# WHU-USI3DV/LaneMapping

Measured on AMD Instinct MI355X. Metric: BEV tiles/sec end-to-end (LAS points -> polylines), higher is better.
Workload: dtype f32; 1 GPU; on-GPU LAS->BEV raster (4,194,304 points/tile resident in HBM) + configs/Proj_polyline_fpn_vit_vertex_2.py, batch=16 per GPU, seeded random weights; lines_per_tile=45, streams=2, hip_graphs=True, points=resident, stream_check=not run (--full runs it), gather_check=n/a (1 rank), raster_check=not run (--full runs it), dist_ranks=1, rccl_ranks=1

## Files before the change

### include/lanemap_hip.h

```cpp
#ifndef LANEMAP_HIP_H
#define LANEMAP_HIP_H
#include <stdint.h>
#ifdef __cplusplus
extern "C" {
#endif

enum { LM_OK = 0, LM_ERR_ARG = 1, LM_ERR_HIP = 2, LM_ERR_NO_DEVICE = 3, LM_ERR_CAPACITY = 4 };
enum { LM_ACT_NONE = 0, LM_ACT_RELU = 1, LM_ACT_GELU = 2 };

int lm_abi_version(void);
const char* lm_last_error(void);
int lm_device_count(void);

int lm_conv2d_nhwc_mfma_f32(void* stream, const float* x, int ldx, const float* wp, int CoutP,
                            const float* scale, const float* shift, const float* res, int ldr, int res_rows,
                            float* y, int ldy, int B, int H, int W, int Cin, int Cout, int KH, int KW,
                            int stride, int pad_h, int pad_w, int dil, int act);
int lm_conv2d_nhwc_mfma_resup_f32(void* stream, const float* x, int ldx, const float* wp, int CoutP, const float* scale,
                                  const float* shift, const float* res_coarse, int ldr, int Hr, int Wr, float* y, int ldy,
                                  int B, int H, int W, int Cin, int Cout, int KH, int KW, int stride, int pad_h, int pad_w,
                                  int dil, int act);

int lm_winograd44_supported(int H, int W, int Cin, int dil);
int lm_winograd44_gn_chunks(int H, int W, int dil);
// ... 4 lines not shown
                              int Cin, int Cout, int dil, int act, double* gn_partial);
int lm_conv3x3_winograd44_twin_f32(void* stream, const float* x, int ldx, const float* wu, int CoutP, const float* scale,
                                   const float* shift, const float* res, int ldr, float* y, int ldy, int B, int H, int W,
                                   int Cin, int Cout, int dil, int act, void* workspace, long workspace_bytes);
int lm_wino44_split_fragments(void* stream, const float* frag, float* out, long n_quads);
int lm_conv3x3_winograd44_split_f32(void* stream, const float* x, int ldx, const float* wu_split, int CoutP, const float* scale,
                                    const float* shift, const float* res, int ldr, float* y, int ldy, int B, int H, int W,
                                    int Cin, int Cout, int dil, int act, double* gn_partial, float post);
int lm_conv3x3_winograd44_split_twin_f32(void* stream, const float* x, int ldx, const float* wu, int CoutP, const float* scale,
                                         const float* shift, const float* res, int ldr, float* y, int ldy, int B, int H, int W,
                                         int Cin, int Cout, int dil, int act, void* workspace, long workspace_bytes, float post);

int lm_conv2d_nhwc_mfma_f32_gnstats(void* stream, const float* x, int ldx, const float* wp, int CoutP, const float* shift,
                                    float* y, int ldy, double* gn_partial, int B, int H, int W, int Cin, int Cout,
                                    int KH, int KW, int stride, int pad_h, int pad_w, int dil);
int lm_gn_finalize(void* stream, const double* partial, float* stats, int B, int HW, int C, int nchunk, float eps);
int lm_gn_finalize_split(void* stream, const double* partial, float* stats, int B, int HW, int C, int nchunk, float eps, int split);

int lm_stem_conv7x7_bn_relu(void* stream, const float* x_chw, const float* w_k64, const float* scale,
                            const float* shift, float* y_nhwc, int B, int H, int W);
int lm_stem_conv7x7_bn_relu_u8(void* stream, const unsigned char* x_hwc3, const float* w_k64, const float* scale,
                               const float* shift, float* y_nhwc, int B, int H, int W);
int lm_maxpool3x3s2_nhwc(void* stream, const float* x, float* y, int B, int H, int W, int C);
int lm_conv2d_nhwc_small(void* stream, const float* x, int ldx, const float* w_tc16, const float* scale,
                         const float* shift, float* y, int ldy, int B, int H, int W, int Cin, int Cout,
                         int KH, int KW, int stride, int pad_h, int pad_w, int pre_relu, int act);

int lm_gn_stats(void* stream, const float* x, double* workspace, float* stats, int B, int HW, int C, float eps);
long lm_gn_stats_workspace_bytes(int B, int HW, int C);
int lm_gn_relu_upsample(void* stream, const float* x, const float* stats, const float* gamma, const float* beta,
                        float* y, int B, int Hi, int Wi, int Ho, int Wo, int C, int accumulate);
int lm_gn_relu_upsample_sum(void* stream, int n, const float* const* x, const float* const* stats, const int* Hi, const int* Wi,
                            const int* ldx , const float* gamma, const float* beta,
                            float* y, int B, int Ho, int Wo, int C);
int lm_gn_relu_upsample_sum_conv1x1(void* stream, int n, const float* const* x, const float* const* stats, const int* Hi, const int* Wi,
                                    const int* ldx, const float* gamma, const float* beta, float* y, int B, int Ho, int Wo, int C,
                                    const float* w_c16, const float* bias, int cout, float* y1, int ldy1);
int lm_upsample_bilinear_nhwc(void* stream, const float* x, int ldx, const float* add, int lda, float* y, int ldy,
                              int B, int Hi, int Wi, int Ho, int Wo, int C);
int lm_upsample_bilinear_to_chw(void* stream, const float* x, int ldx, float* y_chw, int B, int Hi, int Wi,
                                int Ho, int Wo, int C);
int lm_layernorm_rows(void* stream, const float* x, const float* gamma, const float* beta, float* y,
                      long rows, int D, float eps);
int lm_unpatchify(void* stream, const float* tokens, float* y_nhwc, int B, int G, int P, int C);
int lm_token_mix_mfma_f32(void* stream, const float* x, const float* wt, int ldw, const float* bias, const float* res, float* y,
                          int B, int M, int K, int N, int act);
// ... 142 lines not shown
```

### lanemapping_amd/_lib.py

```python
import ctypes as C
import os

_HERE = os.path.dirname(os.path.abspath(__file__))
LIB_PATH = os.environ.get('LANEMAP_HIP_LIB') or os.path.join(_HERE, 'liblanemap_hip.so')

c_f32p = C.POINTER(C.c_float)
vp, i32, i64, f32 = C.c_void_p, C.c_int, C.c_long, C.c_float


class LmRasterParams(C.Structure):
    _fields_ = [('quat', C.c_float * 4), ('trans', C.c_float * 3), ('bev_img_offset', C.c_float * 2),
                ('img_reso', C.c_float * 2), ('local_min_ele', C.c_float), ('ele_reso', C.c_float),
                ('inten_lo', C.c_float), ('inten_hi', C.c_float)]


class LmLasHeader(C.Structure):
    _fields_ = [('version_major', C.c_int), ('version_minor', C.c_int), ('point_format', C.c_int), ('record_len', C.c_int),
                ('n_points', C.c_long), ('offset_to_points', C.c_long), ('scale', C.c_double * 3), ('offset', C.c_double * 3),
                ('min_xyz', C.c_double * 3), ('max_xyz', C.c_double * 3)]


class LmStripGrid(C.Structure):
    _fields_ = [('x0', C.c_double), ('y0', C.c_double), ('cell', C.c_double), ('nx', C.c_int), ('ny', C.c_int)]

# ... 5 lines not shown
SIGNATURES = {
    'lm_abi_version': (i32, []),
    'lm_last_error': (C.c_char_p, []),
    'lm_device_count': (i32, []),
    'lm_conv2d_nhwc_mfma_f32': (i32, [vp, vp, i32, vp, i32, vp, vp, vp, i32, i32, vp, i32,
                                      i32, i32, i32, i32, i32, i32, i32, i32, i32, i32, i32, i32]),
    'lm_conv2d_nhwc_mfma_resup_f32': (i32, [vp, vp, i32, vp, i32, vp, vp, vp, i32, i32, i32, vp, i32,
                                            i32, i32, i32, i32, i32, i32, i32, i32, i32, i32, i32, i32]),
    'lm_winograd44_supported': (i32, [i32, i32, i32, i32]),
    'lm_winograd44_gn_chunks': (i32, [i32, i32, i32]),
    'lm_winograd44_tiles': (i64, [i32, i32, i32, i32]),
    'lm_winograd44_twin_workspace_bytes': (i64, [i32, i32, i32, i32, i32, i32]),
    'lm_conv3x3_winograd44_f32': (i32, [vp, vp, i32, vp, i32, vp, vp, vp, i32, vp, i32, i32, i32, i32, i32, i32, i32, i32, vp]),
    'lm_conv3x3_winograd44_twin_f32': (i32, [vp, vp, i32, vp, i32, vp, vp, vp, i32, vp, i32, i32, i32, i32, i32, i32, i32, i32, vp, i64]),
    'lm_wino44_split_fragments': (i32, [vp, vp, vp, i64]),
    'lm_conv3x3_winograd44_split_f32': (i32, [vp, vp, i32, vp, i32, vp, vp, vp, i32, vp, i32, i32, i32, i32, i32, i32, i32, i32, vp, f32]),
    'lm_conv3x3_winograd44_split_twin_f32': (i32, [vp, vp, i32, vp, i32, vp, vp, vp, i32, vp, i32, i32, i32, i32, i32, i32, i32, i32, vp, i64, f32]),
    'lm_conv2d_nhwc_mfma_f32_gnstats': (i32, [vp, vp, i32, vp, i32, vp, vp, i32, vp] + [i32] * 11),
    'lm_gn_finalize': (i32, [vp, vp, vp, i32, i32, i32, i32, f32]),
    'lm_gn_finalize_split': (i32, [vp, vp, vp, i32, i32, i32, i32, f32, i32]),
    'lm_stem_conv7x7_bn_relu': (i32, [vp, vp, vp, vp, vp, vp, i32, i32, i32]),
    'lm_stem_conv7x7_bn_relu_u8': (i32, [vp, vp, vp, vp, vp, vp, i32, i32, i32]),
    'lm_maxpool3x3s2_nhwc': (i32, [vp, vp, vp, i32, i32, i32, i32]),
    'lm_conv2d_nhwc_small': (i32, [vp, vp, i32, vp, vp, vp, vp, i32, i32, i32, i32, i32, i32, i32, i32, i32, i32, i32, i32, i32]),
    'lm_gn_stats': (i32, [vp, vp, vp, vp, i32, i32, i32, f32]),
    'lm_gn_stats_workspace_bytes': (i64, [i32, i32, i32]),
    'lm_gn_relu_upsample': (i32, [vp, vp, vp, vp, vp, vp, i32, i32, i32, i32, i32, i32, i32]),
    'lm_gn_relu_upsample_sum': (i32, [vp, i32, vp, vp, vp, vp, vp, vp, vp, vp, i32, i32, i32, i32]),
    'lm_gn_relu_upsample_sum_conv1x1': (i32, [vp, i32, vp, vp, vp, vp, vp, vp, vp, vp, i32, i32, i32, i32, vp, vp, i32, vp, i32]),
    'lm_upsample_bilinear_nhwc': (i32, [vp, vp, i32, vp, i32, vp, i32, i32, i32, i32, i32, i32, i32]),
    'lm_upsample_bilinear_to_chw': (i32, [vp, vp, i32, vp, i32, i32, i32, i32, i32, i32]),
    'lm_layernorm_rows': (i32, [vp, vp, vp, vp, vp, i64, i32, f32]),
    'lm_token_mix_mfma_f32': (i32, [vp, vp, vp, i32, vp, vp, vp, i32, i32, i32, i32, i32]),
    'lm_unpatchify': (i32, [vp, vp, vp, i32, i32, i32, i32]),
    'lm_attention_f32': (i32, [vp, vp, vp, i32, i32, i32, i32, f32]),
    'lm_attention_masked_f32': (i32, [vp, vp, vp, vp, i32, i32, i32, i32, f32]),
    'lm_head_tokens': (i32, [vp, vp, vp, vp, f32, i32, i32, i32, i32, i32, i32]),
    'lm_head_tokens_window': (i32, [vp, vp, vp, i32, i32, i32, i32, i32, i32]),
    'lm_head_stage2': (i32, [vp, vp, i32, i32, vp, vp, vp, vp, vp, i64]),
    'lm_head_proposal_conf': (i32, [vp, vp, vp, vp, vp, i32, i32]),
    'lm_head_endpoint_tile': (i32, []),
    'lm_head_endpoint': (i32, [vp, vp, i32, vp, vp, vp, vp, vp, vp, vp, vp, i32, i32, i32, i32, i32]),
    'lm_decode_proposals': (i32, [vp, vp, vp, vp, vp, vp, vp, vp, vp, vp, i32, i32, i32, f32, i32, i32]),
    'lm_decode_orient': (i32, [vp, vp, i32, i32, vp, i64]),
    'lm_decode_semantic': (i32, [vp, vp, vp, vp, vp, i32, i32, i32, f32, i32]),
    'lm_endp_topk_workspace_bytes': (i64, [i32]),
# ... 85 lines not shown
```

### lanemapping_amd/csrc/conv_direct.hip

```cpp
#include "common.h"

#include <type_traits>

typedef float f32x4 __attribute__((ext_vector_type(4)));

namespace {

constexpr int ST = 16;
constexpr int SP = 2 * ST + 5;
constexpr int SPP = 40;

template <bool U8>
__global__ __launch_bounds__(256) void stem_kernel(const void* __restrict__ xin, const float* __restrict__ w,
                                                   const float* __restrict__ scale, const float* __restrict__ shift,
                                                   float* __restrict__ y, int H, int W, int Ho, int Wo) {
    __shared__ float in[3][SP][SPP];
    const int tid = threadIdx.x;
    const int b = blockIdx.z;
    const int oy0 = blockIdx.y * ST, ox0 = blockIdx.x * ST;
    const int iy0 = oy0 * 2 - 3, ix0 = ox0 * 2 - 3;
    for (int i = tid; i < 3 * SP * SP; i += 256) {
        const int c = i / (SP * SP), r = (i / SP) % SP, q = i % SP;
        const int iy = iy0 + r, ix = ix0 + q;
        float v = 0.f;
// ... 14 lines not shown
            for (int c = 0; c < 3; ++c) {
                const float v = in[c][2 * py + ky][2 * px + kx];
                const float* wr = w + ((ky * 7 + kx) * 3 + c) * 64;
#pragma unroll
                for (int q = 0; q < 64; ++q) acc[q] = fmaf(v, wr[q], acc[q]);
            }
    const int oy = oy0 + py, ox = ox0 + px;
    if (oy < Ho && ox < Wo) {
        f32x4* out = reinterpret_cast<f32x4*>(y + (((long)b * Ho + oy) * Wo + ox) * 64);
#pragma unroll
        for (int q = 0; q < 16; ++q) {
            f32x4 o;
#pragma unroll
            for (int e = 0; e < 4; ++e) o[e] = fmaxf(acc[4 * q + e] * scale[4 * q + e] + shift[4 * q + e], 0.f);
            out[q] = o;
        }
    }
}

constexpr int SMW = 112;
constexpr int SMJ = 77;
typedef float f32x16s __attribute__((ext_vector_type(16)));

template <bool U8>
__global__ __launch_bounds__(256, 2) void stem_mfma_kernel(const void* __restrict__ xin, const float* __restrict__ w,
                                                           const float* __restrict__ scale, const float* __restrict__ shift,
                                                           float* __restrict__ y, int H, int W, int Ho, int Wo, LmFastDiv div_tx, LmFastDiv div_ty,
                                                           int ntiles) {
    __shared__ float in[SP * SMW];
    __shared__ float wl[SMJ * 2 * 64];
    __shared__ float u8lut[256];
    u8lut[threadIdx.x] = (float)threadIdx.x / 255.0f;
    const int tid = threadIdx.x, lane = tid & 63, wave = tid >> 6;
    const int l32 = lane & 31, half = lane >> 5;
    for (int i = tid; i < SMJ * 2 * 64; i += 256) {
        const int j = i >> 7, nb = (i >> 6) & 1, l = i & 63;
        const int ky = (2 * j) / 22, idx = (2 * j) % 22 + (l >> 5);
        wl[i] = idx == 21 ? 0.f : w[(ky * 21 + idx) * 64 + nb * 32 + (l & 31)];
    }
    float sc[2], sh[2];
#pragma unroll
    for (int nb = 0; nb < 2; ++nb) {
        sc[nb] = scale[nb * 32 + l32];
        sh[nb] = shift[nb * 32 + l32];
    }
    int abase[2];
#pragma unroll
    for (int mb = 0; mb < 2; ++mb) abase[mb] = (2 * (4 * wave + 2 * mb + (l32 >> 4))) * SMW + (2 * (l32 & 15)) * 3 + half;
    constexpr int NST = (SP * SMW + 255) / 256;
    int poff[NST], prq[NST];
#pragma unroll
    for (int k = 0; k < NST; ++k) {
        const int i = tid + k * 256;
// ... 47 lines not shown
            for (int nb = 0; nb < 2; ++nb)
#pragma unroll
                for (int r = 0; r < 16; ++r) acc[mb][nb][r] = 0.f;
        float av[2][2], wv[2][2];
        auto rd = [&](int j, float (&a)[2], float (&wq)[2]) {
            const int koff = ((2 * j) / 22) * SMW + (2 * j) % 22;
#pragma unroll
            for (int mb = 0; mb < 2; ++mb) a[mb] = in[abase[mb] + koff];
#pragma unroll
            for (int nb = 0; nb < 2; ++nb) wq[nb] = wl[(j * 2 + nb) * 64 + lane];
        };
        rd(0, av[0], wv[0]);
#pragma unroll
        for (int j = 0; j < SMJ; ++j) {
            if (j + 1 < SMJ) rd(j + 1, av[(j + 1) & 1], wv[(j + 1) & 1]);
            __builtin_amdgcn_sched_barrier(0);
#pragma unroll
            for (int mb = 0; mb < 2; ++mb)
#pragma unroll
                for (int nb = 0; nb < 2; ++nb)
                    acc[mb][nb] = __builtin_amdgcn_mfma_f32_32x32x2f32(av[j & 1][mb], wv[j & 1][nb], acc[mb][nb], 0, 0, 0);
            __builtin_amdgcn_sched_barrier(0);
        }
        float* const yt = y + (((long)b * Ho + oy0) * Wo + ox0) * 64;
        const unsigned lbyte = (unsigned)((4 * wave * Wo + 4 * half) * 64 + l32) << 2;
        auto store_tile = [&](auto guarded) {
#pragma unroll
            for (int mb = 0; mb < 2; ++mb)
#pragma unroll
                for (int r = 0; r < 16; ++r) {
                    const int ry = 2 * mb + (r >> 3), cx = (r & 3) + 8 * ((r >> 2) & 1);
                    char* const rowp = reinterpret_cast<char*>(yt) + (long)((ry * Wo + cx) * 64) * 4;
                    if (!decltype(guarded)::value || (oy0 + 4 * wave + ry < Ho && ox0 + cx + 4 * half < Wo)) {
#pragma unroll
                        for (int nb = 0; nb < 2; ++nb)
                            *reinterpret_cast<float*>(rowp + nb * 128 + lbyte) = fmaxf(acc[mb][nb][r] * sc[nb] + sh[nb], 0.f);
                    }
                }
        };
        if (oy0 + ST <= Ho && ox0 + ST <= Wo) store_tile(std::false_type{});
        else store_tile(std::true_type{});
    }
}

__global__ __launch_bounds__(256) void maxpool3x3s2_kernel(const float* __restrict__ x, float* __restrict__ y,
                                                           int H, int W, int C, int Ho, int Wo, long total4) {
    const long i = (long)blockIdx.x * 256 + threadIdx.x;
    if (i >= total4) return;
    const int c4 = C / 4;
    const int c = (int)(i % c4);
    long t = i / c4;
    const int ox = (int)(t % Wo);
    t /= Wo;
    const int oy = (int)(t % Ho);
    const int b = (int)(t / Ho);
    f32x4 m = {-INFINITY, -INFINITY, -INFINITY, -INFINITY};
#pragma unroll
    for (int dy = 0; dy < 3; ++dy)
#pragma unroll
        for (int dx = 0; dx < 3; ++dx) {
            const int iy = oy * 2 - 1 + dy, ix = ox * 2 - 1 + dx;
            if ((unsigned)iy < (unsigned)H && (unsigned)ix < (unsigned)W) {
                const f32x4 v = *reinterpret_cast<const f32x4*>(x + (((long)b * H + iy) * W + ix) * C + c * 4);
#pragma unroll
                for (int e = 0; e < 4; ++e) m[e] = fmaxf(m[e], v[e]);
// ... 46 lines not shown
#pragma unroll
    for (int n = 0; n < 16; ++n) {
        if (n < p.Cout) {
            float v = acc[n];
            if (p.scale) v *= p.scale[n];
            if (p.shift) v += p.shift[n];
            if (p.act == LM_ACT_RELU) v = fmaxf(v, 0.f);
            yp[n] = v;
        }
    }
}

template <bool U8>
int launch_stem(void* stream, const void* x, const float* w_k64, const float* scale, const float* shift, float* y, int B, int H, int W, int Ho,
                int Wo) {
    static const bool valu = [] { const char* e = getenv("LM_STEM_VALU"); return e && atoi(e) != 0; }();
    const int tx = lm_cdiv(Wo, ST), ty = lm_cdiv(Ho, ST);
    if (valu) {
        hipLaunchKernelGGL(stem_kernel<U8>, dim3(tx, ty, B), dim3(256), 0, (hipStream_t)stream, x, w_k64, scale, shift, y, H, W, Ho, Wo);
    } else {
        const long ntiles = (long)tx * ty * B;
        LM_REQUIRE(ntiles < (1L << 31), "stem: too many tiles");
        const int grid = (int)(ntiles < 512 ? ntiles : 512);
        hipLaunchKernelGGL(stem_mfma_kernel<U8>, dim3(grid), dim3(256), 0, (hipStream_t)stream, x, w_k64, scale, shift, y, H, W, Ho, Wo,
                           lm_fastdiv_make((unsigned)tx), lm_fastdiv_make((unsigned)ty), (int)ntiles);
    }
    LM_LAUNCH_CHECK();
    return LM_OK;
}

template <int STRIDE>
__global__ __launch_bounds__(256) void small_conv3x3_mfma_kernel(SmallConvParams p, LmFastDiv div_tx, LmFastDiv div_ty, int ntiles) {
    constexpr int R = 15 * STRIDE + 3;
    extern __shared__ __attribute__((aligned(16))) float patch[];
    const int tid = threadIdx.x, lane = tid & 63, wave = tid >> 6;
    const int l16 = lane & 15, h = lane >> 4;
    float wr[9][4];
#pragma unroll
    for (int t = 0; t < 9; ++t)
#pragma unroll
        for (int j = 0; j < 4; ++j) wr[t][j] = p.w[(t * 16 + 4 * j + h) * 16 + l16];
    float sc = 1.f, sh = 0.f;
    const bool has_sc = p.scale != nullptr, has_sh = p.shift != nullptr;
    if (has_sc && l16 < p.Cout) sc = p.scale[l16];
    if (has_sh && l16 < p.Cout) sh = p.shift[l16];
    for (int t = blockIdx.x; t < ntiles; t += gridDim.x) {
        const unsigned trow = lm_fastdiv((unsigned)t, div_tx);
        const int b = (int)lm_fastdiv(trow, div_ty);
        const int oy0 = (int)(trow - (unsigned)b * div_ty.d) * 16, ox0 = (int)((unsigned)t - trow * div_tx.d) * 16;
        const int iy0 = oy0 * STRIDE - 1, ix0 = ox0 * STRIDE - 1;
// ... 189 lines not shown
    }
}

int launch_small_wide(const SmallConvParams& p, hipStream_t stream) {
    const bool s1 = p.stride == 1;
    if (p.Cin == 8) return s1 ? launch_small_mfma_wide_nb<1, 8>(p, stream) : launch_small_mfma_wide_nb<2, 8>(p, stream);
    return s1 ? launch_small_mfma_wide_nb<1, 16>(p, stream) : launch_small_mfma_wide_nb<2, 16>(p, stream);
}

}

LM_API int lm_stem_conv7x7_bn_relu(void* stream, const float* x_chw, const float* w_k64, const float* scale,
                                   const float* shift, float* y_nhwc, int B, int H, int W) {
    LM_REQUIRE(x_chw && w_k64 && scale && shift && y_nhwc, "stem: null pointer");
    const int Ho = (H + 6 - 7) / 2 + 1, Wo = (W + 6 - 7) / 2 + 1;
    return launch_stem<false>(stream, (const void*)x_chw, w_k64, scale, shift, y_nhwc, B, H, W, Ho, Wo);
}

LM_API int lm_stem_conv7x7_bn_relu_u8(void* stream, const unsigned char* x_hwc3, const float* w_k64, const float* scale,
                                      const float* shift, float* y_nhwc, int B, int H, int W) {
    LM_REQUIRE(x_hwc3 && w_k64 && scale && shift && y_nhwc, "stem_u8: null pointer");
    const int Ho = (H + 6 - 7) / 2 + 1, Wo = (W + 6 - 7) / 2 + 1;
    return launch_stem<true>(stream, (const void*)x_hwc3, w_k64, scale, shift, y_nhwc, B, H, W, Ho, Wo);
}

LM_API int lm_maxpool3x3s2_nhwc(void* stream, const float* x, float* y, int B, int H, int W, int C) {
    LM_REQUIRE(x && y && C % 4 == 0, "maxpool: bad args (C=%d)", C);
    const int Ho = (H + 2 - 3) / 2 + 1, Wo = (W + 2 - 3) / 2 + 1;
    const long total4 = (long)B * Ho * Wo * (C / 4);
    hipLaunchKernelGGL(maxpool3x3s2_kernel, dim3(lm_cdiv(total4, 256)), dim3(256), 0, (hipStream_t)stream,
                       x, y, H, W, C, Ho, Wo, total4);
    LM_LAUNCH_CHECK();
    return LM_OK;
}

LM_API int lm_conv2d_nhwc_small(void* stream, const float* x, int ldx, const float* w_tc16, const float* scale,
                                const float* shift, float* y, int ldy, int B, int H, int W, int Cin, int Cout,
                                int KH, int KW, int stride, int pad_h, int pad_w, int pre_relu, int act) {
    LM_REQUIRE(x && w_tc16 && y, "small_conv: null pointer");
    LM_REQUIRE(Cin % 4 == 0 && ldx % 4 == 0 && Cout >= 1 && (Cout <= 16 || (Cout <= 64 && Cout % 16 == 0)),
               "small_conv: Cin=%d (mult of 4) Cout=%d (<= 16, or 32 / 48 / 64)", Cin, Cout);
    SmallConvParams p;
    p.x = x; p.w = w_tc16; p.scale = scale; p.shift = shift; p.y = y;
    p.ldx = ldx; p.ldy = ldy; p.B = B; p.H = H; p.W = W; p.Cin = Cin; p.Cout = Cout;
    p.KH = KH; p.KW = KW; p.stride = stride; p.pad_h = pad_h; p.pad_w = pad_w; p.pre_relu = pre_relu; p.act = act;
    p.Ho = (H + 2 * pad_h - KH) / stride + 1;
// ... 26 lines not shown
```

### lanemapping_amd/ops.py

```python
import ctypes as C
import math

import torch

from ._lib import lib, check, LmRasterParams, LmStripGrid, LanemapHipError

ACT_NONE, ACT_RELU, ACT_GELU = 0, 1, 2


def _stream():
    return C.c_void_p(torch._C._cuda_getCurrentRawStream(torch._C._cuda_getDevice()))


def _ptr(t):
    if t is None:
        return None
    if not t.is_cuda:
        raise LanemapHipError('lanemapping_amd ops need tensors on an MI355X (HIP) device; no CPU fallback exists')
    if t.device.index != torch._C._cuda_getDevice():
        raise LanemapHipError(f'tensor on cuda:{t.device.index} but the current device is cuda:{torch._C._cuda_getDevice()}: '
                              'call torch.cuda.set_device() (one process drives one GPU)')
    return C.c_void_p(t.data_ptr())


# ... 269 lines not shown
    ph, pw = (pad, pad) if isinstance(pad, int) else pad
    Ho = (H + 2 * ph - kh) // stride + 1
    Wo = (W + 2 * pw - kw) // stride + 1
    if out is None:
        out = new_act(B, cout, Ho, Wo, x.device)
    out_, ldy = as_nhwc(out)
    assert out_.data_ptr() == out.data_ptr()
    check(lib().lm_conv2d_nhwc_small(_stream(), _ptr(x), ldx, _ptr(w16), _ptr(scale), _ptr(shift), _ptr(out), ldy,
                                     B, H, W, cin, cout, kh, kw, stride, ph, pw, int(pre_relu), act))
    return out


def stem(x, w_k64, scale, shift):
    x = x.contiguous()
    if x.dtype == torch.uint8:
        B, H, W, C_ = x.shape
        assert C_ == 3, 'u8 tiles are [B,H,W,3]'
    else:
        B, _, H, W = x.shape
    Ho, Wo = (H - 1) // 2 + 1, (W - 1) // 2 + 1
    out = new_act(B, 64, Ho, Wo, x.device)
    fn = lib().lm_stem_conv7x7_bn_relu_u8 if x.dtype == torch.uint8 else lib().lm_stem_conv7x7_bn_relu
    check(fn(_stream(), _ptr(x), _ptr(w_k64), _ptr(scale), _ptr(shift), _ptr(out), B, H, W))
    return out


def maxpool3x3s2(x):
    x, ld = as_nhwc(x)
    B, C_, H, W = x.shape
    assert ld == C_
    out = new_act(B, C_, (H - 1) // 2 + 1, (W - 1) // 2 + 1, x.device)
    check(lib().lm_maxpool3x3s2_nhwc(_stream(), _ptr(x), _ptr(out), B, H, W, C_))
    return out


def gn_stats(x, eps=1e-5):
    x, ld = as_nhwc(x)
    B, C_, H, W = x.shape
    assert ld == C_
    ws = torch.empty(lib().lm_gn_stats_workspace_bytes(B, H * W, C_) // 8, device=x.device, dtype=torch.float64)
    stats = torch.empty((B, C_, 2), device=x.device, dtype=torch.float32)
    check(lib().lm_gn_stats(_stream(), _ptr(x), _ptr(ws), _ptr(stats), B, H * W, C_, eps))
    return stats


def gn_relu_upsample(x, stats, gamma, beta, size, out=None, accumulate=False):
# ... 481 lines not shown
```

### lanemapping_amd/pcencoder.py

```python
import os

import torch
import torch.nn as nn

from . import ops, trace
from .registry import PCENCODER
from .packing import PackedModule

_LAYERS = {'resnet18': [2, 2, 2, 2], 'resnet34': [3, 4, 6, 3]}
MERGE_BRANCH_CONVS = os.environ.get('LANEMAP_MERGE_BRANCH_CONVS', '1') != '0'
WINO_F44 = os.environ.get('LANEMAP_WINO_F44', '1') != '0'
WINO_F44_MIN_CIN = int(os.environ.get('LANEMAP_WINO_F44_MIN_CIN', '64'))
WINO_SPLIT = os.environ.get('LANEMAP_WINO_SPLIT', '0') != '0'


def _frag44(w):
    if WINO_SPLIT:
        return ops.pack_wino44_fragments_split(ops.pack_wino44(w))
    return ops.pack_wino44_fragments(ops.pack_wino44(w))


def _f44_ok(conv):
    return WINO_F44 and conv.kernel_size == (3, 3) and conv.stride == (1, 1) and conv.in_channels >= WINO_F44_MIN_CIN and conv.in_channels % 16 == 0


class _ResBlock(nn.Module):

    def __init__(self, cin, cout, stride, dilation, with_down):
        super().__init__()
        self.conv1 = nn.Conv2d(cin, cout, 3, stride, dilation, dilation, bias=False)
        self.bn1 = nn.BatchNorm2d(cout)
        self.conv2 = nn.Conv2d(cout, cout, 3, 1, dilation, dilation, bias=False)
        self.bn2 = nn.BatchNorm2d(cout)
        self.downsample = nn.Sequential(nn.Conv2d(cin, cout, 1, stride, bias=False), nn.BatchNorm2d(cout)) if with_down else None
        self.stride, self.dilation = stride, dilation

# ... 142 lines not shown
        s4 = ops.gn_relu_upsample_sum([(t, st)], P[gn_a + '.g'], P[gn_a + '.b'], (h, w))
        terms = [pre[0] if pre is not None and pre[0] is not None else self._conv_stats(P, p2, conv_b, c_half, gn_b),
                 pre[1] if pre is not None and pre[1] is not None else self._conv_stats(P, p3, conv_b, c_half, gn_b)]
        terms.append(self._conv_stats(P, s4, conv_b, c_half, gn_b))
        return ops.gn_relu_upsample_sum(terms, P[gn_b + '.g'], P[gn_b + '.b'], (h, w), proj=proj, keep_sum=False)

    def forward(self, x, fea_up_out=None):
        from . import torch_ops
        if self.out is None:
            return self._forward_impl(x, fea_up_out)
        if fea_up_out is None:
            B, H, W = (x.shape[0], x.shape[1], x.shape[2]) if x.dtype == torch.uint8 else (x.shape[0], x.shape[2], x.shape[3])
            fea_up_out = ops.new_act(B, 8, (H + 3) // 4, (W + 3) // 4, x.device)
        fea, bi_seg, endp = torch_ops.fpn_encoder(x, fea_up_out, torch_ops.stage_weights(self), torch_ops.stage_name(self))
        return fea, fea_up_out, bi_seg, endp

    def _forward_impl(self, x, fea_up_out=None):
        P = self.packed()
        if x.dtype == torch.uint8:
            B, H, W, _ = x.shape
        else:
            B, _, H, W = x.shape
        with trace.stage('fpn.stem'):
            c1 = ops.maxpool3x3s2(ops.stem(x, P['stem_w'], P['stem_s'], P['stem_b']))
        feats = []
        t = c1
        for lname in ('layer1', 'layer2', 'layer3'):
            with trace.stage('fpn.' + lname):
                for i, blk in enumerate(getattr(self, lname)):
                    t = self._block(t, P, f'{lname}.{i}', blk)
            feats.append(t)
        c2, c3, c4 = feats
        trace.push('fpn.topdown')
        fea = ops.conv_mfma(c4, P['out.w'], self.out.out_channels) if self.out is not None else None
        p4 = ops.conv_mfma(c4, P['toplayer.w'], 256, shift=P['toplayer.b'])
        def lateral(c, name, coarse):
            if tuple(coarse.shape[2:]) == tuple(c.shape[2:]):
                return ops.conv_mfma(c, P[name + '.w'], 256, shift=P[name + '.b'], res=coarse)
            return ops.conv_mfma(c, P[name + '.w'], 256, shift=P[name + '.b'], res_up=coarse)

        p3 = lateral(c3, 'latlayer1', p4)
        p2 = lateral(c2, 'latlayer2', p3)
        del c1, c2, c3, c4, feats, t
        p4 = self._conv3(p4, P, 'smooth1', 256)
        p3 = self._conv3(p3, P, 'smooth2', 256)
        p2 = self._conv3(p2, P, 'smooth3', 256)
        trace.pop()
# ... 41 lines not shown
```

### lanemapping_amd/torch_ops.py

```python
import itertools
import weakref
from typing import List, Optional, Tuple

import numpy as np
import torch
from torch import Tensor

from . import ops as _ops

_STAGES = weakref.WeakValueDictionary()
_STAGE_COUNTER = itertools.count()


def stage_name(module):
    n = module.__dict__.get('_lanemap_stage_name')
    if n is None:
        n = module.__dict__['_lanemap_stage_name'] = f'{type(module).__name__}#{next(_STAGE_COUNTER)}'
    _STAGES[n] = module
    return n


def stage_weights(module):
    return [d[n] for d, n in module._slots() if d[n] is not None]

# ... 52 lines not shown
def _conv2d_mfma_fake(x, w_packed, cout, kh, kw, stride, pad, dil, scale, shift, res, act):
    Ho, Wo = _out_hw(x.shape[2], x.shape[3], kh, kw, stride, pad, dil)
    return _fake_act(x, x.shape[0], cout, Ho, Wo)


def _conv3x3_winograd44(x: Tensor, wu_frag: Tensor, cout: int, dil: int, scale: Optional[Tensor], shift: Optional[Tensor],
                        res: Optional[Tensor], act: int) -> Tensor:
    return _ops.conv_wino44(x, wu_frag, cout, dil, scale=scale, shift=shift, res=res, act=act)


def _conv3x3_fake(x, w, cout, dil, scale, shift, res, act):
    return _fake_act(x, x.shape[0], cout, x.shape[2], x.shape[3])


def _stem(x: Tensor, w_k64: Tensor, scale: Tensor, shift: Tensor) -> Tensor:
    return _ops.stem(x, w_k64, scale, shift)


def _stem_fake(x, w_k64, scale, shift):
    B, H, W = (x.shape[0], x.shape[1], x.shape[2]) if x.dtype == torch.uint8 else (x.shape[0], x.shape[2], x.shape[3])
    return _fake_act(x, B, 64, (H - 1) // 2 + 1, (W - 1) // 2 + 1)


def _maxpool(x: Tensor) -> Tensor:
    return _ops.maxpool3x3s2(x)


def _maxpool_fake(x):
    return _fake_act(x, x.shape[0], x.shape[1], (x.shape[2] - 1) // 2 + 1, (x.shape[3] - 1) // 2 + 1)


def _gn_stats(x: Tensor, eps: float) -> Tensor:
    return _ops.gn_stats(x, eps)


def _gn_stats_fake(x, eps):
    return x.new_empty((x.shape[0], x.shape[1], 2))


def _gn_relu_upsample(x: Tensor, stats: Tensor, gamma: Tensor, beta: Tensor, Ho: int, Wo: int) -> Tensor:
    return _ops.gn_relu_upsample(x, stats, gamma, beta, (Ho, Wo))


def _upsample_bilinear(x: Tensor, Ho: int, Wo: int) -> Tensor:
    y = _ops.upsample_nhwc(x, (Ho, Wo))
    return y.clone() if y.data_ptr() == x.data_ptr() else y
# ... 40 lines not shown


def _decode_semantic_fake(logits, thre):
    B, _, H, W = logits.shape
    return logits.new_empty((B, H, W), dtype=torch.uint8), logits.new_empty((B, H, W)), logits.new_empty((B, H // 8, W))


def _decode_orient(orient_logits: Tensor) -> Tensor:
    return _ops.decode_orient(orient_logits)


def _endp_topk(endp_logits: Tensor, K: int, clip: int) -> Tuple[Tensor, Tensor, Tensor]:
    return _ops.endp_topk(endp_logits, K=K, clip=clip)


def _endp_topk_fake(endp_logits, K, clip):
    B = endp_logits.shape[0]
    return (endp_logits.new_empty((B, K), dtype=torch.int32), endp_logits.new_empty((B, K)), endp_logits.new_empty((B,), dtype=torch.int32))


conv2d_mfma = _define('conv2d_mfma', _conv2d_mfma, _conv2d_mfma_fake)
conv3x3_winograd44 = _define('conv3x3_winograd44', _conv3x3_winograd44, _conv3x3_fake)
stem_conv7x7 = _define('stem_conv7x7', _stem, _stem_fake)
maxpool3x3s2 = _define('maxpool3x3s2', _maxpool, _maxpool_fake)
gn_stats = _define('gn_stats', _gn_stats, _gn_stats_fake)
gn_relu_upsample = _define('gn_relu_upsample', _gn_relu_upsample, lambda x, stats, gamma, beta, Ho, Wo: _resize_fake(x, Ho, Wo))
upsample_bilinear = _define('upsample_bilinear', _upsample_bilinear, lambda x, Ho, Wo: _resize_fake(x, Ho, Wo))
layernorm_rows = _define('layernorm_rows', _layernorm_rows, lambda x, gamma, beta, eps: torch.empty_like(x))
attention = _define('attention', _attention, lambda qkv, B, N, heads, dim_head, scale: qkv.new_empty((B * N, heads * dim_head)))
linear_mfma = _define('linear_mfma', _linear_mfma,
                      lambda x, w_packed, n_out, scale, shift, res, res_rows, act: x.new_empty((x.shape[0], n_out)))
token_mix = _define('token_mix', _token_mix, lambda x, wt, M, bias, B, res, act: x.new_empty((B * M, x.shape[1])))
tile_ingest = _define('tile_ingest', _tile_ingest,
                      lambda u8: u8.new_empty((u8.shape[0], 3, u8.shape[1], u8.shape[2]), dtype=torch.float32))
decode_proposals = _define('decode_proposals', _decode_proposals, _decode_proposals_fake)
decode_semantic = _define('decode_semantic', _decode_semantic, _decode_semantic_fake)
decode_orient = _define('decode_orient', _decode_orient,
                        lambda o: o.new_empty((o.shape[0], o.shape[2], o.shape[3]), dtype=torch.uint8))
endp_topk = _define('endp_topk', _endp_topk, _endp_topk_fake)


def _bev_raster(points: Tensor, tile_offsets: List[int], params: Tensor, H: int, W: int) -> Tensor:
    p = params.detach().cpu().float().numpy()
    pars = [_ops.make_raster_params(quat=r[0:4], trans=r[4:7], bev_img_offset=r[7:9], img_reso=r[9:11], local_min_ele=r[11],
                                    ele_reso=r[12], inten_lo=r[13], inten_hi=r[14]) for r in p]
    return _ops.bev_raster_batch(points, tile_offsets, pars, H, W, u8_only=True)
# ... 90 lines not shown
    n = torch.library.get_ctx().new_dynamic_size()
    return topk_idx.new_empty((n, 2), dtype=torch.int32)


endp_cluster = _define('endp_cluster', _endp_cluster, _endp_cluster_fake, device='cpu')


def _polyline_assemble(prop_conf: Tensor, prop_v_ext: Tensor, cls_offset: Tensor, bi_seg_rows: Tensor, endp_hw: Tensor,
                       obj_thre: float) -> Tuple[Tensor, Tensor]:
    from . import hostpost
    lanes, kept = hostpost.assemble_polylines(prop_conf.numpy(), prop_v_ext.numpy(), cls_offset.numpy(), bi_seg_rows.numpy(),
                                              endp_hw.numpy(), obj_thre)
    return torch.from_numpy(lanes), torch.from_numpy(np.ascontiguousarray(kept, dtype=np.int32).reshape(-1, 2))


def _polyline_assemble_fake(prop_conf, prop_v_ext, cls_offset, bi_seg_rows, endp_hw, obj_thre):
    n = torch.library.get_ctx().new_dynamic_size()
    P, R = prop_v_ext.shape
    return prop_conf.new_empty((P, R, 2), dtype=torch.float64), endp_hw.new_empty((n, 2), dtype=torch.int32)


polyline_assemble = _define('polyline_assemble', _polyline_assemble, _polyline_assemble_fake, device='cpu')

OP_NAMES = ['conv2d_mfma', 'conv3x3_winograd44', 'stem_conv7x7', 'maxpool3x3s2', 'gn_stats', 'gn_relu_upsample',
            'upsample_bilinear', 'layernorm_rows', 'attention', 'linear_mfma', 'token_mix', 'tile_ingest', 'decode_proposals', 'decode_semantic',
            'decode_orient', 'endp_topk', 'bev_raster', 'fpn_encoder', 'vit_backbone', 'mixer_backbone', 'colprop_head', 'colprop_endpoint', 'endp_cluster', 'polyline_assemble']
```

Baseline: 372.4 tiles/s.

## Fuse 3x3 stride-2 maxpool into stem conv7x7 epilogue with seam fixup kernel

Adds a pooled variant of the MFMA stem kernel that applies BN+ReLU and a 3x3/s2 max pool inside each 8x8 output tile. It uses shuffles and shared memory to cover neighbours within the tile. Tile-boundary rows and columns go to a workspace, and a small seam kernel merges them into the pooled output. This removes the full-resolution 64-channel stem activation write and its re-read by a separate maxpool kernel. The cost is a second launch, a per-call workspace allocation, and more complex epilogue logic. The new path is on by default through LANEMAP_STEM_POOL.

```diff
diff --git a/include/lanemap_hip.h b/include/lanemap_hip.h
--- a/include/lanemap_hip.h
+++ b/include/lanemap_hip.h
@@ -50,6 +50,11 @@
 int lm_stem_conv7x7_bn_relu_u8(void* stream, const unsigned char* x_hwc3, const float* w_k64, const float* scale,
                                const float* shift, float* y_nhwc, int B, int H, int W);
 int lm_maxpool3x3s2_nhwc(void* stream, const float* x, float* y, int B, int H, int W, int C);
+long lm_stem_pool_workspace_bytes(int B, int H, int W);
+int lm_stem_pool_conv7x7_bn_relu(void* hip_stream, const float* x_chw, const float* w_k64, const float* scale, const float* shift,
+                                 float* y_nhwc, void* workspace, long workspace_bytes, int B, int H, int W);
+int lm_stem_pool_conv7x7_bn_relu_u8(void* hip_stream, const unsigned char* x_hwc3, const float* w_k64, const float* scale,
+                                    const float* shift, float* y_nhwc, void* workspace, long workspace_bytes, int B, int H, int W);
 int lm_conv2d_nhwc_small(void* stream, const float* x, int ldx, const float* w_tc16, const float* scale,
                          const float* shift, float* y, int ldy, int B, int H, int W, int Cin, int Cout,
                          int KH, int KW, int stride, int pad_h, int pad_w, int pre_relu, int act);
diff --git a/lanemapping_amd/_lib.py b/lanemapping_amd/_lib.py
--- a/lanemapping_amd/_lib.py
+++ b/lanemapping_amd/_lib.py
@@ -51,6 +51,9 @@
     'lm_stem_conv7x7_bn_relu': (i32, [vp, vp, vp, vp, vp, vp, i32, i32, i32]),
     'lm_stem_conv7x7_bn_relu_u8': (i32, [vp, vp, vp, vp, vp, vp, i32, i32, i32]),
     'lm_maxpool3x3s2_nhwc': (i32, [vp, vp, vp, i32, i32, i32, i32]),
+    'lm_stem_pool_workspace_bytes': (i64, [i32, i32, i32]),
+    'lm_stem_pool_conv7x7_bn_relu': (i32, [vp, vp, vp, vp, vp, vp, vp, i64, i32, i32, i32]),
+    'lm_stem_pool_conv7x7_bn_relu_u8': (i32, [vp, vp, vp, vp, vp, vp, vp, i64, i32, i32, i32]),
     'lm_conv2d_nhwc_small': (i32, [vp, vp, i32, vp, vp, vp, vp, i32, i32, i32, i32, i32, i32, i32, i32, i32, i32, i32, i32, i32]),
     'lm_gn_stats': (i32, [vp, vp, vp, vp, i32, i32, i32, f32]),
     'lm_gn_stats_workspace_bytes': (i64, [i32, i32, i32]),
diff --git a/lanemapping_amd/csrc/conv_direct.hip b/lanemapping_amd/csrc/conv_direct.hip
--- a/lanemapping_amd/csrc/conv_direct.hip
+++ b/lanemapping_amd/csrc/conv_direct.hip
@@ -60,13 +60,19 @@
 constexpr int SMJ = 77;
 typedef float f32x16s __attribute__((ext_vector_type(16)));
 
-template <bool U8>
+struct StemPoolOut {
+    float* rowbuf; float* colbuf;
+    int Hp, Wp, ntx, nty;
+};
+
+template <bool U8, bool POOL>
 __global__ __launch_bounds__(256, 2) void stem_mfma_kernel(const void* __restrict__ xin, const float* __restrict__ w,
                                                            const float* __restrict__ scale, const float* __restrict__ shift,
                                                            float* __restrict__ y, int H, int W, int Ho, int Wo, LmFastDiv div_tx, LmFastDiv div_ty,
-                                                           int ntiles) {
+                                                           int ntiles, StemPoolOut po) {
     __shared__ float in[SP * SMW];
     __shared__ float wl[SMJ * 2 * 64];
+    __shared__ float xch[POOL ? 3 * 2 * 4 * 64 : 1];
     __shared__ float u8lut[256];
     u8lut[threadIdx.x] = (float)threadIdx.x / 255.0f;
     const int tid = threadIdx.x, lane = tid & 63, wave = tid >> 6;
@@ -160,6 +166,63 @@
                     acc[mb][nb] = __builtin_amdgcn_mfma_f32_32x32x2f32(av[j & 1][mb], wv[j & 1][nb], acc[mb][nb], 0, 0, 0);
             __builtin_amdgcn_sched_barrier(0);
         }
+        if constexpr (POOL) {
+            const int ty = oy0 / ST, tx = ox0 / ST;
+            const bool side_row = wave == 3 && ty + 1 < po.nty, side_col = half == 1 && tx + 1 < po.ntx;
+            float* const rowp = po.rowbuf + (((long)b * (po.nty - 1) + ty) * Wo + ox0) * 64 + l32;
+            float* const colp = po.colbuf + (((long)b * (po.ntx - 1) + tx) * Ho + oy0 + 4 * wave) * 64 + l32;
+            float* const yp = y + (((long)b * po.Hp + oy0 / 2 + 2 * wave) * po.Wp + ox0 / 2 + 2 * half) * 64 + l32;
+            auto pool_tile = [&](auto guarded) {
+                constexpr bool G = decltype(guarded)::value;
+                float hm[2][4][4];
+#pragma unroll
+                for (int R = 0; R < 4; ++R) {
+                    const int mb = R >> 1, rr = R & 1;
+                    const bool rowok = !G || oy0 + 4 * wave + R < Ho;
+#pragma unroll
+                    for (int nb = 0; nb < 2; ++nb) {
+                        float v[8];
+#pragma unroll
+                        for (int i = 0; i < 8; ++i) {
+                            const int cx = (i & 3) + 8 * (i >> 2) + 4 * half;
+                            const bool ok = rowok && (!G || ox0 + cx < Wo);
+                            const float val = fmaxf(acc[mb][nb][8 * rr + i] * sc[nb] + sh[nb], 0.f);
+                            v[i] = ok ? val : -INFINITY;
+                            if (R == 3 && side_row && ok) rowp[cx * 64 + nb * 32] = val;
+                        }
+                        if (side_col && rowok) colp[R * 64 + nb * 32] = v[7];
+                        const float x3 = __shfl_xor(v[3], 32), x7 = __shfl_xor(v[7], 32);
+                        const float l0 = half ? x3 : -INFINITY, l1 = half ? x7 : x3;
+                        hm[nb][R][0] = fmaxf(fmaxf(l0, v[0]), v[1]);
+                        hm[nb][R][1] = fmaxf(fmaxf(v[1], v[2]), v[3]);
+                        hm[nb][R][2] = fmaxf(fmaxf(l1, v[4]), v[5]);
+                        hm[nb][R][3] = fmaxf(fmaxf(v[5], v[6]), v[7]);
+                    }
+                }
+                if (wave < 3) {
+#pragma unroll
+                    for (int nb = 0; nb < 2; ++nb)
+#pragma unroll
+                        for (int p = 0; p < 4; ++p) xch[((wave * 2 + nb) * 4 + p) * 64 + lane] = hm[nb][3][p];
+                }
+                __syncthreads();
+#pragma unroll
+                for (int nb = 0; nb < 2; ++nb)
+#pragma unroll
+                    for (int p = 0; p < 4; ++p) {
+                        const float above = wave > 0 ? xch[(((wave - 1) * 2 + nb) * 4 + p) * 64 + lane] : -INFINITY;
+                        const float m0 = fmaxf(fmaxf(above, hm[nb][0][p]), hm[nb][1][p]);
+                        const float m1 = fmaxf(fmaxf(hm[nb][1][p], hm[nb][2][p]), hm[nb][3][p]);
+                        const int pc = (p & 1) + 4 * (p >> 1);
+                        const bool cok = !G || ox0 / 2 + 2 * half + pc < po.Wp;
+                        if (cok && (!G || oy0 / 2 + 2 * wave < po.Hp)) yp[pc * 64 + nb * 32] = m0;
+                        if (cok && (!G || oy0 / 2 + 2 * wave + 1 < po.Hp)) yp[(po.Wp + pc) * 64 + nb * 32] = m1;
+                    }
+            };
+            if (oy0 + ST <= Ho && ox0 + ST <= Wo) pool_tile(std::false_type{});
+            else pool_tile(std::true_type{});
+            continue;
+        }
         float* const yt = y + (((long)b * Ho + oy0) * Wo + ox0) * 64;
         const unsigned lbyte = (unsigned)((4 * wave * Wo + 4 * half) * 64 + l32) << 2;
         auto store_tile = [&](auto guarded) {
@@ -179,6 +242,53 @@
         if (oy0 + ST <= Ho && ox0 + ST <= Wo) store_tile(std::false_type{});
         else store_tile(std::true_type{});
     }
+}
+
+__global__ __launch_bounds__(256) void stem_pool_seam_kernel(float* __restrict__ y, const float* __restrict__ rowbuf,
+                                                             const float* __restrict__ colbuf, int Ho, int Wo, StemPoolOut po, long total) {
+    const long i = (long)blockIdx.x * 256 + threadIdx.x;
+    if (i >= total) return;
+    const int c = (int)(i & 15);
+    const long t = i >> 4;
+    const int nrow = (po.nty - 1) * po.Wp, per = nrow + (po.ntx - 1) * po.Hp;
+    const int b = (int)(t / per);
+    int k = (int)(t - (long)b * per), py, px;
+    if (k < nrow) {
+        py = 8 * (k / po.Wp + 1);
+        px = k % po.Wp;
+    } else {
+        k -= nrow;
+        px = 8 * (k / po.Hp + 1);
+        py = k % po.Hp;
+        if ((py & 7) == 0 && py > 0) return;
+    }
+    f32x4* const out = reinterpret_cast<f32x4*>(y + (((long)b * po.Hp + py) * po.Wp + px) * 64 + c * 4);
+    f32x4 m = *out;
+    if ((py & 7) == 0 && py > 0) {
+        const float* const row = rowbuf + ((long)b * (po.nty - 1) + (py / 8 - 1)) * Wo * 64 + c * 4;
+#pragma unroll
+        for (int dx = -1; dx <= 1; ++dx) {
+            const int ix = 2 * px + dx;
+            if ((unsigned)ix < (unsigned)Wo) {
+                const f32x4 v = *reinterpret_cast<const f32x4*>(row + (long)ix * 64);
+#pragma unroll
+                for (int e = 0; e < 4; ++e) m[e] = fmaxf(m[e], v[e]);
+            }
+        }
+    }
+    if ((px & 7) == 0 && px > 0) {
+        const float* const col = colbuf + ((long)b * (po.ntx - 1) + (px / 8 - 1)) * Ho * 64 + c * 4;
+#pragma unroll
+        for (int dy = -1; dy <= 1; ++dy) {
+            const int iy = 2 * py + dy;
+            if ((unsigned)iy < (unsigned)Ho) {
+                const f32x4 v = *reinterpret_cast<const f32x4*>(col + (long)iy * 64);
+#pragma unroll
+                for (int e = 0; e < 4; ++e) m[e] = fmaxf(m[e], v[e]);
+            }
+        }
+    }
+    *out = m;
 }
 
 __global__ __launch_bounds__(256) void maxpool3x3s2_kernel(const float* __restrict__ x, float* __restrict__ y,
@@ -271,10 +381,45 @@
         const long ntiles = (long)tx * ty * B;
         LM_REQUIRE(ntiles < (1L << 31), "stem: too many tiles");
         const int grid = (int)(ntiles < 512 ? ntiles : 512);
-        hipLaunchKernelGGL(stem_mfma_kernel<U8>, dim3(grid), dim3(256), 0, (hipStream_t)stream, x, w_k64, scale, shift, y, H, W, Ho, Wo,
-                           lm_fastdiv_make((unsigned)tx), lm_fastdiv_make((unsigned)ty), (int)ntiles);
+        hipLaunchKernelGGL((stem_mfma_kernel<U8, false>), dim3(grid), dim3(256), 0, (hipStream_t)stream, x, w_k64, scale, shift, y, H, W, Ho, Wo,
+                           lm_fastdiv_make((unsigned)tx), lm_fastdiv_make((unsigned)ty), (int)ntiles, StemPoolOut{});
     }
     LM_LAUNCH_CHECK();
+    return LM_OK;
+}
+
+long stem_pool_side_floats(int B, int Ho, int Wo, long* col_off) {
+    const long rows = (long)B * (lm_cdiv(Ho, ST) - 1) * Wo * 64, cols = (long)B * (lm_cdiv(Wo, ST) - 1) * Ho * 64;
+    if (col_off) *col_off = rows;
+    return rows + cols;
+}
+
+template <bool U8>
+int launch_stem_pool(void* stream, const void* x, const float* w_k64, const float* scale, const float* shift, float* y, void* workspace,
+                     long workspace_bytes, int B, int H, int W) {
+    LM_REQUIRE(B >= 1 && H >= 1 && W >= 1 && H < (1 << 15) && W < (1 << 15), "stem_pool: bad shape B=%d H=%d W=%d", B, H, W);
+    const int Ho = (H + 6 - 7) / 2 + 1, Wo = (W + 6 - 7) / 2 + 1;
+    long col_off;
+    const long need = stem_pool_side_floats(B, Ho, Wo, &col_off) * 4;
+    LM_REQUIRE(workspace_bytes >= need && (workspace || need == 0), "stem_pool: workspace of %ld bytes, need %ld", workspace_bytes, need);
+    StemPoolOut po;
+    po.rowbuf = static_cast<float*>(workspace);
+    po.colbuf = po.rowbuf + col_off;
+    po.Hp = (Ho + 1) / 2; po.Wp = (Wo + 1) / 2;
+    po.ntx = lm_cdiv(Wo, ST); po.nty = lm_cdiv(Ho, ST);
+    const long ntiles = (long)po.ntx * po.nty * B;
+    LM_REQUIRE(ntiles < (1L << 31), "stem_pool: too many tiles");
+    const int grid = (int)(ntiles < 512 ? ntiles : 512);
+    hipLaunchKernelGGL((stem_mfma_kernel<U8, true>), dim3(grid), dim3(256), 0, (hipStream_t)stream, x, w_k64, scale, shift, y, H, W, Ho, Wo,
+                       lm_fastdiv_make((unsigned)po.ntx), lm_fastdiv_make((unsigned)po.nty), (int)ntiles, po);
+    LM_LAUNCH_CHECK();
+    const long total = (long)B * ((long)(po.nty - 1) * po.Wp + (long)(po.ntx - 1) * po.Hp) * 16;
+    if (total > 0) {
+        LM_REQUIRE(lm_cdiv(total, 256) > 0, "stem_pool: too many seam pixels");
+        hipLaunchKernelGGL(stem_pool_seam_kernel, dim3(lm_cdiv(total, 256)), dim3(256), 0, (hipStream_t)stream, y, po.rowbuf, po.colbuf, Ho, Wo,
+                           po, total);
+        LM_LAUNCH_CHECK();
+    }
     return LM_OK;
 }
 
@@ -510,6 +655,23 @@
     LM_REQUIRE(x_hwc3 && w_k64 && scale && shift && y_nhwc, "stem_u8: null pointer");
     const int Ho = (H + 6 - 7) / 2 + 1, Wo = (W + 6 - 7) / 2 + 1;
     return launch_stem<true>(stream, (const void*)x_hwc3, w_k64, scale, shift, y_nhwc, B, H, W, Ho, Wo);
+}
+
+LM_API long lm_stem_pool_workspace_bytes(int B, int H, int W) {
+    if (B < 1 || H < 1 || W < 1) return 0;
+    return stem_pool_side_floats(B, (H + 6 - 7) / 2 + 1, (W + 6 - 7) / 2 + 1, nullptr) * 4;
+}
+
+LM_API int lm_stem_pool_conv7x7_bn_relu(void* hip_stream, const float* x_chw, const float* w_k64, const float* scale, const float* shift,
+                                        float* y_nhwc, void* workspace, long workspace_bytes, int B, int H, int W) {
+    LM_REQUIRE(x_chw && w_k64 && scale && shift && y_nhwc, "stem_pool: null pointer");
+    return launch_stem_pool<false>(hip_stream, (const void*)x_chw, w_k64, scale, shift, y_nhwc, workspace, workspace_bytes, B, H, W);
+}
+
+LM_API int lm_stem_pool_conv7x7_bn_relu_u8(void* hip_stream, const unsigned char* x_hwc3, const float* w_k64, const float* scale,
+                                           const float* shift, float* y_nhwc, void* workspace, long workspace_bytes, int B, int H, int W) {
+    LM_REQUIRE(x_hwc3 && w_k64 && scale && shift && y_nhwc, "stem_pool_u8: null pointer");
+    return launch_stem_pool<true>(hip_stream, (const void*)x_hwc3, w_k64, scale, shift, y_nhwc, workspace, workspace_bytes, B, H, W);
 }
 
 LM_API int lm_maxpool3x3s2_nhwc(void* stream, const float* x, float* y, int B, int H, int W, int C) {
diff --git a/lanemapping_amd/ops.py b/lanemapping_amd/ops.py
--- a/lanemapping_amd/ops.py
+++ b/lanemapping_amd/ops.py
@@ -315,6 +315,22 @@
     out = new_act(B, 64, Ho, Wo, x.device)
     fn = lib().lm_stem_conv7x7_bn_relu_u8 if x.dtype == torch.uint8 else lib().lm_stem_conv7x7_bn_relu
     check(fn(_stream(), _ptr(x), _ptr(w_k64), _ptr(scale), _ptr(shift), _ptr(out), B, H, W))
+    return out
+
+
+def stem_pool(x, w_k64, scale, shift):
+    x = x.contiguous()
+    if x.dtype == torch.uint8:
+        B, H, W, C_ = x.shape
+        assert C_ == 3, 'u8 tiles are [B,H,W,3]'
+    else:
+        B, _, H, W = x.shape
+    Ho, Wo = (H - 1) // 2 + 1, (W - 1) // 2 + 1
+    out = new_act(B, 64, (Ho - 1) // 2 + 1, (Wo - 1) // 2 + 1, x.device)
+    need = lib().lm_stem_pool_workspace_bytes(B, H, W)
+    ws = torch.empty(need, device=x.device, dtype=torch.uint8)
+    fn = lib().lm_stem_pool_conv7x7_bn_relu_u8 if x.dtype == torch.uint8 else lib().lm_stem_pool_conv7x7_bn_relu
+    check(fn(_stream(), _ptr(x), _ptr(w_k64), _ptr(scale), _ptr(shift), _ptr(out), _ptr(ws), need, B, H, W))
     return out
 
 
diff --git a/lanemapping_amd/pcencoder.py b/lanemapping_amd/pcencoder.py
--- a/lanemapping_amd/pcencoder.py
+++ b/lanemapping_amd/pcencoder.py
@@ -12,6 +12,7 @@
 WINO_F44 = os.environ.get('LANEMAP_WINO_F44', '1') != '0'
 WINO_F44_MIN_CIN = int(os.environ.get('LANEMAP_WINO_F44_MIN_CIN', '64'))
 WINO_SPLIT = os.environ.get('LANEMAP_WINO_SPLIT', '0') != '0'
+STEM_POOL = os.environ.get('LANEMAP_STEM_POOL', '1') != '0'
 
 
 def _frag44(w):
@@ -200,7 +201,10 @@
         else:
             B, _, H, W = x.shape
         with trace.stage('fpn.stem'):
-            c1 = ops.maxpool3x3s2(ops.stem(x, P['stem_w'], P['stem_s'], P['stem_b']))
+            if STEM_POOL:
+                c1 = ops.stem_pool(x, P['stem_w'], P['stem_s'], P['stem_b'])
+            else:
+                c1 = ops.maxpool3x3s2(ops.stem(x, P['stem_w'], P['stem_s'], P['stem_b']))
         feats = []
         t = c1
         for lname in ('layer1', 'layer2', 'layer3'):
diff --git a/lanemapping_amd/torch_ops.py b/lanemapping_amd/torch_ops.py
--- a/lanemapping_amd/torch_ops.py
+++ b/lanemapping_amd/torch_ops.py
@@ -98,6 +98,16 @@
     return _fake_act(x, B, 64, (H - 1) // 2 + 1, (W - 1) // 2 + 1)
 
 
+def _stem_pool(x: Tensor, w_k64: Tensor, scale: Tensor, shift: Tensor) -> Tensor:
+    return _ops.stem_pool(x, w_k64, scale, shift)
+
+
+def _stem_pool_fake(x, w_k64, scale, shift):
+    B, H, W = (x.shape[0], x.shape[1], x.shape[2]) if x.dtype == torch.uint8 else (x.shape[0], x.shape[2], x.shape[3])
+    Ho, Wo = (H - 1) // 2 + 1, (W - 1) // 2 + 1
+    return _fake_act(x, B, 64, (Ho - 1) // 2 + 1, (Wo - 1) // 2 + 1)
+
+
 def _maxpool(x: Tensor) -> Tensor:
     return _ops.maxpool3x3s2(x)
 
@@ -184,6 +194,7 @@
 conv2d_mfma = _define('conv2d_mfma', _conv2d_mfma, _conv2d_mfma_fake)
 conv3x3_winograd44 = _define('conv3x3_winograd44', _conv3x3_winograd44, _conv3x3_fake)
 stem_conv7x7 = _define('stem_conv7x7', _stem, _stem_fake)
+stem_pool_conv7x7 = _define('stem_pool_conv7x7', _stem_pool, _stem_pool_fake)
 maxpool3x3s2 = _define('maxpool3x3s2', _maxpool, _maxpool_fake)
 gn_stats = _define('gn_stats', _gn_stats, _gn_stats_fake)
 gn_relu_upsample = _define('gn_relu_upsample', _gn_relu_upsample, lambda x, stats, gamma, beta, Ho, Wo: _resize_fake(x, Ho, Wo))
@@ -320,6 +331,6 @@
 
 polyline_assemble = _define('polyline_assemble', _polyline_assemble, _polyline_assemble_fake, device='cpu')
 
-OP_NAMES = ['conv2d_mfma', 'conv3x3_winograd44', 'stem_conv7x7', 'maxpool3x3s2', 'gn_stats', 'gn_relu_upsample',
+OP_NAMES = ['conv2d_mfma', 'conv3x3_winograd44', 'stem_conv7x7', 'stem_pool_conv7x7', 'maxpool3x3s2', 'gn_stats', 'gn_relu_upsample',
             'upsample_bilinear', 'layernorm_rows', 'attention', 'linear_mfma', 'token_mix', 'tile_ingest', 'decode_proposals', 'decode_semantic',
             'decode_orient', 'endp_topk', 'bev_raster', 'fpn_encoder', 'vit_backbone', 'mixer_backbone', 'colprop_head', 'colprop_endpoint', 'endp_cluster', 'polyline_assemble']
```

Result: slower. 364.5 tiles/s (-2.1%).
